# lxa9867/ImageFolder

Hardware: NVIDIA H100
Metric: tokenizer_train_images_per_sec_256x256 (higher is better)
Workload: dtype bf16

## Files before the change

imagefolder_b200/csrc/attn_kernel.cu:

```cuda
#include "xq_common.cuh"
#include "xq_tc.cuh"

#include <mutex>

namespace xq {
using namespace xqtc;

constexpr int AT_BM = 128;
constexpr int AT_BN = 128;
constexpr int AT_D = 64;
constexpr int AT_NS = 2;
constexpr int AT_TILE = AT_BM * AT_D * 2;
constexpr int AT_THREADS = 288;

struct AttnFwdSmem {
    static constexpr int Q = 0;
    static constexpr int K = AT_TILE;
    static constexpr int V = AT_TILE * (1 + AT_NS);
    static constexpr int BAR = AT_TILE * (1 + 2 * AT_NS);
    static constexpr int BYTES = BAR + 256;
};

__device__ __forceinline__ void named_bar_sync(int id, int nthreads) { asm volatile("bar.sync %0, %1;" ::"r"(id), "r"(nthreads) : "memory"); }

__global__ void __launch_bounds__(AT_THREADS, 1)
attn_fwd_kernel(const __grid_constant__ CUtensorMap tmQKV, __nv_bfloat16 *__restrict__ out, float *__restrict__ lse2, int N, int H,
                int nQ , float c ) {
    extern __shared__ uint8_t smem_raw[];
    uint8_t *base = (uint8_t *)(((uintptr_t)smem_raw + 1023) & ~(uintptr_t)1023);
    uint64_t *bars = (uint64_t *)(base + AttnFwdSmem::BAR);
    uint64_t *q_full = bars + 0;
    uint64_t *k_full = bars + 1;
    uint64_t *k_empty = bars + 1 + AT_NS;
    uint64_t *v_full = bars + 1 + 2 * AT_NS;
// ... 22 lines not shown
        for (int j = 0; j < nK; ++j) {
            const int st = j % AT_NS;
            const uint32_t ph = ((j / AT_NS) & 1) ^ 1;
            mbar_wait(&k_empty[st], ph);
            if (elect_one()) {
                mbar_expect_tx(&k_full[st], AT_TILE);
                tma_load_3d(base + AttnFwdSmem::K + st * AT_TILE, &tmQKV, colK, j * AT_BN, b, &k_full[st]);
            }
            __syncwarp();
            mbar_wait(&v_empty[st], ph);
            if (elect_one()) {
                mbar_expect_tx(&v_full[st], AT_TILE);
                tma_load_3d(base + AttnFwdSmem::V + st * AT_TILE, &tmQKV, colV, j * AT_BN, b, &v_full[st]);
            }
            __syncwarp();
        }
        return;
    }

    const int wg = warp >> 2, wq = warp & 3;
    const int rq = wg * 64 + wq * 16 + (lane >> 2), cq = 2 * (lane & 3);
    const uint64_t qd = desc_k_sw128(smem_u32(base + AttnFwdSmem::Q + wg * (AT_TILE / 2)));
    float m[2] = {-CUDART_INF_F, -CUDART_INF_F}, l[2] = {0.f, 0.f};
    float o[32];
#pragma unroll
    for (int i = 0; i < 32; ++i) o[i] = 0.f;
    mbar_wait(q_full, 0);
    for (int j = 0; j < nK; ++j) {
        const int st = j % AT_NS;
        const uint32_t ph = (j / AT_NS) & 1;
        float s[64];
        mbar_wait(&k_full[st], ph);
        const uint64_t kd = desc_k_sw128(smem_u32(base + AttnFwdSmem::K + st * AT_TILE));
        wgmma_fence();
#pragma unroll
        for (int k = 0; k < AT_D / 16; ++k) wgmma_m64n128k16_ss<0, 0>(s, desc_adv(qd, k * 32), desc_adv(kd, k * 32), (uint32_t)k);
        wgmma_commit();
        wgmma_wait<0>();
        fence_regs(s);
        __syncwarp();
        if (lane == 0) mbar_arrive(&k_empty[st]);
        const int nv = N - j * AT_BN;
        if (nv < AT_BN) {
#pragma unroll
            for (int i = 0; i < 64; ++i)
                if (8 * (i >> 2) + cq + (i & 1) >= nv) s[i] = -CUDART_INF_F;
        }
        float mx[2] = {m[0], m[1]};
#pragma unroll
        for (int i = 0; i < 64; ++i) mx[(i >> 1) & 1] = fmaxf(mx[(i >> 1) & 1], s[i]);
#pragma unroll
        for (int hh = 0; hh < 2; ++hh) {
            mx[hh] = fmaxf(mx[hh], __shfl_xor_sync(0xffffffffu, mx[hh], 1));
            mx[hh] = fmaxf(mx[hh], __shfl_xor_sync(0xffffffffu, mx[hh], 2));
        }
        float alpha[2], mc[2];
#pragma unroll
        for (int hh = 0; hh < 2; ++hh) {
            alpha[hh] = ex2_approx((m[hh] - mx[hh]) * c);
            m[hh] = mx[hh];
            mc[hh] = mx[hh] * c;
            l[hh] *= alpha[hh];
        }
#pragma unroll
        for (int i = 0; i < 32; ++i) o[i] *= alpha[(i >> 1) & 1];
        uint32_t pa[AT_BN / 16][4];
#pragma unroll
        for (int i = 0; i < 64; i += 2) {
            const int hh = (i >> 1) & 1;
            const float p0 = ex2_approx(fmaf(s[i], c, -mc[hh])), p1 = ex2_approx(fmaf(s[i + 1], c, -mc[hh]));
            l[hh] += p0 + p1;
            pa[i >> 3][((i >> 2) & 1) * 2 + hh] = pack_bf16(p0, p1);
        }
        mbar_wait(&v_full[st], ph);
        const uint64_t vd = desc_mn_sw128(smem_u32(base + AttnFwdSmem::V + st * AT_TILE), AT_TILE);
        wgmma_fence();
#pragma unroll
        for (int k = 0; k < AT_BN / 16; ++k) wgmma_m64n64k16_rs<1>(o, pa[k], desc_adv(vd, k * 2048), 1u);
        wgmma_commit();
        wgmma_wait<0>();
        fence_regs(o);
        __syncwarp();
        if (lane == 0) mbar_arrive(&v_empty[st]);
    }
#pragma unroll
    for (int hh = 0; hh < 2; ++hh) {
        l[hh] += __shfl_xor_sync(0xffffffffu, l[hh], 1);
        l[hh] += __shfl_xor_sync(0xffffffffu, l[hh], 2);
    }
#pragma unroll
    for (int hh = 0; hh < 2; ++hh) {
        const int n = qt * AT_BM + rq + 8 * hh;
        if (n >= N) continue;
        const float inv = 1.0f / l[hh];
        if (cq == 0) lse2[(size_t)bh * N + n] = fmaf(m[hh], c, log2f(l[hh]));
        __nv_bfloat16 *orow = out + ((size_t)b * N + n) * H * AT_D + h * AT_D;
#pragma unroll
        for (int jj = 0; jj < AT_D / 8; ++jj)
            *reinterpret_cast<uint32_t *>(orow + 8 * jj + cq) = pack_bf16(o[4 * jj + 2 * hh] * inv, o[4 * jj + 2 * hh + 1] * inv);
    }
}

constexpr int AT_TAIL_MAX = 0;

__global__ void __launch_bounds__(128)
attn_fwd_tail_kernel(const __nv_bfloat16 *__restrict__ qkv, __nv_bfloat16 *__restrict__ out, float *__restrict__ lse2, int B, int N,
                     int H, int n0 , float c) {
    const int lane = threadIdx.x & 31;
    const long long w = ((long long)blockIdx.x * blockDim.x + threadIdx.x) >> 5;
    const int nt = N - n0;
    if (w >= (long long)B * H * nt) return;
    const int r = (int)(w % nt);
    const int bh = (int)(w / nt);
    const int b = bh / H, h = bh - b * H;
    const int n = n0 + r;
    const size_t W = (size_t)3 * H * AT_D;
    const __nv_bfloat16 *qp = qkv + ((size_t)b * N + n) * W + h * AT_D;
    float qf[AT_D];
#pragma unroll
    for (int u = 0; u < 8; ++u) {
        const uint4 x = *reinterpret_cast<const uint4 *>(qp + u * 8);
        const __nv_bfloat162 *x2 = reinterpret_cast<const __nv_bfloat162 *>(&x);
#pragma unroll
        for (int e = 0; e < 4; ++e) {
            const float2 f = __bfloat1622float2(x2[e]);
            qf[u * 8 + 2 * e] = f.x * c;
            qf[u * 8 + 2 * e + 1] = f.y * c;
        }
    }
    float m = -CUDART_INF_F, l = 0.f, o[AT_D];
#pragma unroll
    for (int i = 0; i < AT_D; ++i) o[i] = 0.f;
    for (int key = lane; key < N; key += 32) {
        const __nv_bfloat16 *kp = qkv + ((size_t)b * N + key) * W + (H + h) * AT_D;
        const __nv_bfloat16 *vp = kp + (size_t)H * AT_D;
        float s = 0.f;
#pragma unroll
        for (int u = 0; u < 8; ++u) {
            const uint4 x = *reinterpret_cast<const uint4 *>(kp + u * 8);
            const __nv_bfloat162 *x2 = reinterpret_cast<const __nv_bfloat162 *>(&x);
#pragma unroll
            for (int e = 0; e < 4; ++e) {
                const float2 f = __bfloat1622float2(x2[e]);
                s = fmaf(qf[u * 8 + 2 * e], f.x, s);
                s = fmaf(qf[u * 8 + 2 * e + 1], f.y, s);
            }
        }
        const float m_new = fmaxf(m, s);
        const float corr = ex2_approx(m - m_new);
        const float p = ex2_approx(s - m_new);
        l = fmaf(l, corr, p);
        m = m_new;
#pragma unroll
        for (int u = 0; u < 8; ++u) {
            const uint4 x = *reinterpret_cast<const uint4 *>(vp + u * 8);
            const __nv_bfloat162 *x2 = reinterpret_cast<const __nv_bfloat162 *>(&x);
#pragma unroll
            for (int e = 0; e < 4; ++e) {
                const float2 f = __bfloat1622float2(x2[e]);
                o[u * 8 + 2 * e] = fmaf(o[u * 8 + 2 * e], corr, p * f.x);
                o[u * 8 + 2 * e + 1] = fmaf(o[u * 8 + 2 * e + 1], corr, p * f.y);
            }
        }
    }
    float M = m;
#pragma unroll
    for (int off = 16; off > 0; off >>= 1) M = fmaxf(M, __shfl_xor_sync(0xffffffffu, M, off));
    const float f = (m == -CUDART_INF_F) ? 0.f : ex2_approx(m - M);
    l *= f;
#pragma unroll
    for (int off = 16; off > 0; off >>= 1) l += __shfl_xor_sync(0xffffffffu, l, off);
    const float inv = 1.0f / l;
    float mine0 = 0.f, mine1 = 0.f;
#pragma unroll
    for (int i = 0; i < AT_D; ++i) {
        float x = o[i] * f;
#pragma unroll
        for (int off = 16; off > 0; off >>= 1) x += __shfl_xor_sync(0xffffffffu, x, off);
        if (i == 2 * lane) mine0 = x;
        if (i == 2 * lane + 1) mine1 = x;
    }
    __nv_bfloat16 *op = out + ((size_t)b * N + n) * H * AT_D + h * AT_D;
    *reinterpret_cast<uint32_t *>(op + 2 * lane) = pack_bf16(mine0 * inv, mine1 * inv);
    if (lane == 0) lse2[(size_t)bh * N + n] = M + log2f(l);
}

struct AttnMaps {
    const void *qkv;
    int B, N, H;
    CUtensorMap tmQKV;
};

struct AttnDevState { bool fwd_attr = false, bwd_attr = false, prep_attr = false; };
static int attn_dev_state(AttnDevState **out) {
    static std::mutex mu;
    static AttnDevState states[64];
    int dev = 0;
    cudaError_t e = cudaGetDevice(&dev);
    if (e != cudaSuccess) return xq::record_cuda_error(e, "cudaGetDevice");
    if (dev < 0 || dev >= 64) return XQ_ERR_UNSUPPORTED;
    std::lock_guard<std::mutex> g(mu);
    *out = &states[dev];
    return XQ_OK;
}

static bool get_fwd_maps(const void *qkv, int B, int N, int H, AttnMaps &m) {
    static std::mutex mu;
    static AttnMaps cache[16];
    static int n_cached = 0, next = 0;
    std::lock_guard<std::mutex> g(mu);
    for (int i = 0; i < n_cached; ++i)
        if (cache[i].qkv == qkv && cache[i].B == B && cache[i].N == N && cache[i].H == H) { m = cache[i]; return true; }
    AttnMaps e;
    e.qkv = qkv; e.B = B; e.N = N; e.H = H;
    const uint64_t W = (uint64_t)3 * H * AT_D;
    if (!make_map_3d(&e.tmQKV, CU_TENSOR_MAP_DATA_TYPE_BFLOAT16, 2, const_cast<void *>(qkv), W, N, B, W * 2, (uint64_t)N * W * 2, AT_D, AT_BM)) return false;
    cache[next] = e;
    next = (next + 1) % 16;
    if (n_cached < 16) ++n_cached;
    m = e;
    return true;
}


constexpr int AB_THREADS = 288;
constexpr int AB_BQ = 64;
constexpr int AB_QS = 3;
constexpr int AB_QTILE = AB_BQ * AT_D * 2;

struct AttnBwdSmem {
    static constexpr int K = 0;
    static constexpr int V = AT_TILE;
    static constexpr int Q = 2 * AT_TILE;
    static constexpr int DO = Q + AB_QS * AB_QTILE;
    static constexpr int DS = DO + AB_QS * AB_QTILE;
    static constexpr int STAT = DS + 2 * AB_QTILE;
    static constexpr int BAR = STAT + AB_QS * 512;
    static constexpr int BYTES = BAR + 256;
};

__device__ __forceinline__ void bulk_load_1d(void *dst, const void *src, uint32_t bytes, uint64_t *bar) {
    asm volatile("cp.async.bulk.shared::cluster.global.mbarrier::complete_tx::bytes [%0], [%1], %2, [%3];"
                 ::"r"(smem_u32(dst)), "l"(src), "r"(bytes), "r"(smem_u32(bar))
                 : "memory");
}

__device__ __forceinline__ void bwd_epilogue_frag(const float (&acc)[32], float mul, __nv_bfloat16 *__restrict__ row0,
                                                  size_t row_stride, bool ok0, bool ok1, float *__restrict__ g_bias_cols, int lane) {
    const int cq = 2 * (lane & 3);
#pragma unroll
    for (int jj = 0; jj < AT_D / 8; ++jj) {
        const uint32_t w0 = pack_bf16(acc[4 * jj] * mul, acc[4 * jj + 1] * mul);
        const uint32_t w1 = pack_bf16(acc[4 * jj + 2] * mul, acc[4 * jj + 3] * mul);
        if (ok0) *reinterpret_cast<uint32_t *>(row0 + 8 * jj + cq) = w0;
        if (ok1) *reinterpret_cast<uint32_t *>(row0 + 8 * row_stride + 8 * jj + cq) = w1;
        if (g_bias_cols) {
            float s0 = __uint_as_float(w0 << 16) + __uint_as_float(w1 << 16);
            float s1 = __uint_as_float(w0 & 0xffff0000u) + __uint_as_float(w1 & 0xffff0000u);
#pragma unroll
            for (int o = 4; o < 32; o <<= 1) {
                s0 += __shfl_xor_sync(0xffffffffu, s0, o);
                s1 += __shfl_xor_sync(0xffffffffu, s1, o);
            }
            if (lane < 4) {
                atomicAdd(g_bias_cols + 8 * jj + cq, s0);
                atomicAdd(g_bias_cols + 8 * jj + cq + 1, s1);
            }
        }
    }
}

__global__ void __launch_bounds__(AB_THREADS, 1)
attn_bwd_kernel(const __grid_constant__ CUtensorMap tmQKV, const __grid_constant__ CUtensorMap tmDO, const float *__restrict__ lseP,
                const float *__restrict__ deltaP, float *__restrict__ dq_acc, __nv_bfloat16 *__restrict__ dqkv, float *__restrict__ g_bias,
                int N, int H, int Npad, float c, float scale) {
    extern __shared__ uint8_t smem_raw[];
    uint8_t *base = (uint8_t *)(((uintptr_t)smem_raw + 1023) & ~(uintptr_t)1023);
    uint64_t *bars = (uint64_t *)(base + AttnBwdSmem::BAR);
    uint64_t *kv_full = bars;
    uint64_t *q_full = bars + 1;
    uint64_t *q_empty = bars + 1 + AB_QS;
    float *s_lse = (float *)(base + AttnBwdSmem::STAT);
    float *s_delta = s_lse + AB_QS * AB_BQ;

    const int tid = threadIdx.x, warp = tid >> 5, lane = tid & 31;
    const int bh = blockIdx.y, b = bh / H, h = bh - b * H;
    const int k0 = blockIdx.x * AT_BN;
    const int colQ = h * AT_D, colK = (H + h) * AT_D, colV = (2 * H + h) * AT_D;
    const int nQ = (N + AB_BQ - 1) / AB_BQ;

    if (tid == 0) {
        mbar_init(kv_full, 1);
        for (int i = 0; i < AB_QS; ++i) { mbar_init(&q_full[i], 1); mbar_init(&q_empty[i], 8); }
        mbar_fence_init();
    }
    __syncthreads();

// ... 11 lines not shown
        for (int i = 0; i < nQ; ++i) {
            const int st = i % AB_QS;
            mbar_wait(&q_empty[st], ((i / AB_QS) & 1) ^ 1);
            if (elect_one()) {
                mbar_expect_tx(&q_full[st], 2 * AB_QTILE + 2 * AB_BQ * 4);
                tma_load_3d(base + AttnBwdSmem::Q + st * AB_QTILE, &tmQKV, colQ, i * AB_BQ, b, &q_full[st]);
                tma_load_3d(base + AttnBwdSmem::DO + st * AB_QTILE, &tmDO, h * AT_D, i * AB_BQ, b, &q_full[st]);
                bulk_load_1d(s_lse + st * AB_BQ, lseP + (size_t)bh * Npad + i * AB_BQ, AB_BQ * 4, &q_full[st]);
                bulk_load_1d(s_delta + st * AB_BQ, deltaP + (size_t)bh * Npad + i * AB_BQ, AB_BQ * 4, &q_full[st]);
            }
            __syncwarp();
        }
        return;
    }

    const int wg = warp >> 2, wq = warp & 3;
    const int rq = wq * 16 + (lane >> 2), cq = 2 * (lane & 3);
    const int key0 = k0 + wg * 64 + rq;
    const bool kok0 = key0 < N, kok1 = key0 + 8 < N;
    const uint32_t kw = smem_u32(base + AttnBwdSmem::K + wg * AB_QTILE), vw = smem_u32(base + AttnBwdSmem::V + wg * AB_QTILE);
    const uint64_t kd_k = desc_k_sw128(kw), vd_k = desc_k_sw128(vw), kd_mn = desc_mn_sw128(kw, AT_TILE);
    const uint32_t dsw = smem_u32(base + AttnBwdSmem::DS + wg * AB_QTILE);
    const uint64_t dsd = desc_mn_sw128(dsw, AT_TILE);
    float dv[32], dk[32];
#pragma unroll
    for (int i = 0; i < 32; ++i) dv[i] = dk[i] = 0.f;
    mbar_wait(kv_full, 0);
    for (int i = 0; i < nQ; ++i) {
        const int st = i % AB_QS;
        mbar_wait(&q_full[st], (i / AB_QS) & 1);
        const uint32_t qa = smem_u32(base + AttnBwdSmem::Q + st * AB_QTILE), da = smem_u32(base + AttnBwdSmem::DO + st * AB_QTILE);
        float s[32], dp[32];
        wgmma_fence();
#pragma unroll
        for (int k = 0; k < AT_D / 16; ++k) wgmma_m64n64k16_ss<0, 0>(s, desc_adv(kd_k, k * 32), desc_adv(desc_k_sw128(qa), k * 32), (uint32_t)k);
#pragma unroll
        for (int k = 0; k < AT_D / 16; ++k) wgmma_m64n64k16_ss<0, 0>(dp, desc_adv(vd_k, k * 32), desc_adv(desc_k_sw128(da), k * 32), (uint32_t)k);
        wgmma_commit();
        wgmma_wait<0>();
        fence_regs(s);
        fence_regs(dp);
        const float *L = s_lse + st * AB_BQ, *D = s_delta + st * AB_BQ;
        uint32_t pa[4][4], sa[4][4];
#pragma unroll
        for (int jj = 0; jj < AB_BQ / 8; ++jj) {
            const float2 Lq = *reinterpret_cast<const float2 *>(L + 8 * jj + cq);
// ... 11 lines not shown
                sa[jj >> 1][(jj & 1) * 2 + hh] = dw;
                asm volatile("st.shared.b32 [%0], %1;" ::"r"(dsw + rowtile_off_bf16(rq + 8 * hh, 8 * jj + cq)), "r"(dw) : "memory");
            }
        }
        fence_async_smem();
        named_bar_sync(1 + wg, 128);
        const uint64_t qd_mn = desc_mn_sw128(qa, AT_TILE), dd_mn = desc_mn_sw128(da, AT_TILE);
        float dq[32];
        wgmma_fence();
#pragma unroll
        for (int k = 0; k < AB_BQ / 16; ++k) {
            wgmma_m64n64k16_rs<1>(dv, pa[k], desc_adv(dd_mn, k * 2048), 1u);
            wgmma_m64n64k16_rs<1>(dk, sa[k], desc_adv(qd_mn, k * 2048), 1u);
        }
#pragma unroll
        for (int k = 0; k < 64 / 16; ++k) wgmma_m64n64k16_ss<1, 1>(dq, desc_adv(dsd, k * 2048), desc_adv(kd_mn, k * 2048), (uint32_t)k);
        wgmma_commit();
        wgmma_wait<0>();
        fence_regs(dv);
        fence_regs(dk);
        fence_regs(dq);
        __syncwarp();
        if (lane == 0) mbar_arrive(&q_empty[st]);
        named_bar_sync(1 + wg, 128);
#pragma unroll
        for (int hh = 0; hh < 2; ++hh) {
            const int q = i * AB_BQ + rq + 8 * hh;
            if (q < N) {
                float *dst = dq_acc + ((size_t)bh * N + q) * AT_D + cq;
#pragma unroll
                for (int jj = 0; jj < AT_D / 8; ++jj)
                    atomicAdd(reinterpret_cast<float2 *>(dst + 8 * jj), make_float2(dq[4 * jj + 2 * hh], dq[4 * jj + 2 * hh + 1]));
            }
        }
    }
    const size_t W = (size_t)3 * H * AT_D;
    __nv_bfloat16 *row = dqkv + ((size_t)b * N + key0) * W;
    bwd_epilogue_frag(dv, 1.0f, row + colV, W, kok0, kok1, g_bias ? g_bias + colV : nullptr, lane);
    bwd_epilogue_frag(dk, scale, row + colK, W, kok0, kok1, g_bias ? g_bias + colK : nullptr, lane);
}


constexpr int AB_KTAIL_MAX = 4;
constexpr int AB_PREP_ROWS = 128;

__device__ __forceinline__ void unpack8(const uint4 &w, float (&f)[8]) {
    const uint32_t x[4] = {w.x, w.y, w.z, w.w};
#pragma unroll
    for (int e = 0; e < 4; ++e) { f[2 * e] = __uint_as_float(x[e] << 16); f[2 * e + 1] = __uint_as_float(x[e] & 0xffff0000u); }
}

template <int NT>
__global__ void __launch_bounds__(256, 2)
attn_bwd_prep_kernel(const __nv_bfloat16 *__restrict__ qkv, const __nv_bfloat16 *__restrict__ out, const __nv_bfloat16 *__restrict__ dout,
                     const float *__restrict__ lse2, float *__restrict__ lseP, float *__restrict__ deltaP, float *__restrict__ dq_acc,
                     float *__restrict__ dsT, __nv_bfloat16 *__restrict__ dqkv, float *__restrict__ g_bias, int N, int H, int Npad,
                     float c, float scale) {
    constexpr int NTA = NT > 0 ? NT : 1;
// ... 190 lines not shown
        }
    }
    if (!g_bias) return;
#pragma unroll
    for (int e = 0; e < 8; ++e) {
        v[e] += __shfl_xor_sync(0xffffffffu, v[e], 8);
        v[e] += __shfl_xor_sync(0xffffffffu, v[e], 16);
    }
    const int warp = threadIdx.x >> 5, lane = threadIdx.x & 31;
    if (lane < 8) {
#pragma unroll
        for (int e = 0; e < 8; ++e) red[warp][lane * 8 + e] = v[e];
    }
    __syncthreads();
    if (threadIdx.x < AT_D) {
        float acc = 0.f;
#pragma unroll
        for (int w8 = 0; w8 < 8; ++w8) acc += red[w8][threadIdx.x];
        atomicAdd(g_bias + hh * AT_D + threadIdx.x, acc);
    }
}

struct AttnBwdMaps {
    const void *qkv, *dout;
    int B, N, H;
    CUtensorMap tmQKV, tmDO;
};

static bool get_bwd_maps(const void *qkv, const void *dout, int B, int N, int H, AttnBwdMaps &m) {
    static std::mutex mu;
    static AttnBwdMaps cache[16];
    static int n_cached = 0, next = 0;
    std::lock_guard<std::mutex> g(mu);
    for (int i = 0; i < n_cached; ++i)
        if (cache[i].qkv == qkv && cache[i].dout == dout && cache[i].B == B &&
            cache[i].N == N && cache[i].H == H) { m = cache[i]; return true; }
    AttnBwdMaps e;
    e.qkv = qkv; e.dout = dout; e.B = B; e.N = N; e.H = H;
    const uint64_t W = (uint64_t)3 * H * AT_D, Wo = (uint64_t)H * AT_D;
    if (!make_map_3d(&e.tmQKV, CU_TENSOR_MAP_DATA_TYPE_BFLOAT16, 2, const_cast<void *>(qkv), W, N, B, W * 2, (uint64_t)N * W * 2, AT_D, AB_BQ)) return false;
    if (!make_map_3d(&e.tmDO, CU_TENSOR_MAP_DATA_TYPE_BFLOAT16, 2, const_cast<void *>(dout), Wo, N, B, Wo * 2, (uint64_t)N * Wo * 2, AT_D, AB_BQ)) return false;
    cache[next] = e;
    next = (next + 1) % 16;
    if (n_cached < 16) ++n_cached;
    m = e;
    return true;
}

static int attn_bwd_ktail(int N) {
    const int r = N % AT_BN;
    return (N > AT_BN && r != 0 && r <= AB_KTAIL_MAX) ? r : 0;
}

static size_t attn_bwd_ws_layout(int B, int N, int H, size_t *off_lse, size_t *off_delta, size_t *off_dst) {
    const size_t Npad = ((size_t)N + AT_BM - 1) / AT_BM * AT_BM;
    const size_t acc = align_up((size_t)B * H * N * AT_D * sizeof(float), 1024);
    const size_t st = align_up((size_t)B * H * Npad * sizeof(float), 1024);
    const size_t dst = align_up((size_t)B * H * N * attn_bwd_ktail(N) * sizeof(float), 1024);
    if (off_lse) *off_lse = acc;
    if (off_delta) *off_delta = acc + st;
    if (off_dst) *off_dst = acc + 2 * st;
    return acc + 2 * st + dst;
}

// ... 1 lines not shown

extern "C" {

size_t xq_vit_attn_bwd_workspace_bytes(int B, int N, int H) {
    if (B <= 0 || N <= 0 || H <= 0) return 0;
    return xq::attn_bwd_ws_layout(B, N, H, nullptr, nullptr, nullptr);
}

int xq_vit_attn_bwd(const void *qkv, const void *out, const void *d_out, const float *lse2, void *dqkv, float *g_bias, int B, int N,
                    int H, int head_dim, float scale, void *workspace, size_t workspace_bytes, void *stream) {
    using namespace xq;
    if (!qkv || !out || !d_out || !lse2 || !dqkv || !workspace || B <= 0 || N <= 0 || H <= 0) return XQ_ERR_ARG;
    if (head_dim != AT_D) return XQ_ERR_UNSUPPORTED;
    if (((uintptr_t)qkv & 15) || ((uintptr_t)out & 15) || ((uintptr_t)d_out & 15) || ((uintptr_t)dqkv & 15) || ((uintptr_t)workspace & 255))
        return XQ_ERR_ARG;
    size_t off_lse, off_delta, off_dst;
    if (workspace_bytes < attn_bwd_ws_layout(B, N, H, &off_lse, &off_delta, &off_dst)) return XQ_ERR_WORKSPACE;
    cudaStream_t st = (cudaStream_t)stream;
    float *acc = (float *)workspace;
    float *lseP = (float *)((char *)workspace + off_lse);
    float *deltaP = (float *)((char *)workspace + off_delta);
    float *dsT = (float *)((char *)workspace + off_dst);
    AttnBwdMaps m;
    if (!get_bwd_maps(qkv, d_out, B, N, H, m)) return XQ_ERR_UNSUPPORTED;
    const int nt = attn_bwd_ktail(N);
    const int nK = nt ? N / AT_BN : (N + AT_BN - 1) / AT_BN;
    const int Npad = (N + AT_BM - 1) / AT_BM * AT_BM;
    if ((long long)B * H > 65535) return XQ_ERR_UNSUPPORTED;
    if (g_bias) XQ_CUDA_TRY(cudaMemsetAsync(g_bias, 0, (size_t)3 * H * AT_D * sizeof(float), st));
    const float c2 = scale * 1.4426950408889634f;
    AttnDevState *ds = nullptr;
    if (int rc = attn_dev_state(&ds)) return rc;
    {
        dim3 grid(nt ? 1u : (unsigned)(Npad / AB_PREP_ROWS), (unsigned)(B * H));
        const __nv_bfloat16 *qp = (const __nv_bfloat16 *)qkv, *op = (const __nv_bfloat16 *)out, *gp = (const __nv_bfloat16 *)d_out;
        __nv_bfloat16 *dp = (__nv_bfloat16 *)dqkv;
        constexpr int PS = 2 * 3 * (AB_PREP_ROWS / 32) * 256 * 16;
        if (!ds->prep_attr) {
            XQ_CUDA_TRY(cudaFuncSetAttribute(attn_bwd_prep_kernel<1>, cudaFuncAttributeMaxDynamicSharedMemorySize, PS));
            XQ_CUDA_TRY(cudaFuncSetAttribute(attn_bwd_prep_kernel<2>, cudaFuncAttributeMaxDynamicSharedMemorySize, PS));
            XQ_CUDA_TRY(cudaFuncSetAttribute(attn_bwd_prep_kernel<3>, cudaFuncAttributeMaxDynamicSharedMemorySize, PS));
            XQ_CUDA_TRY(cudaFuncSetAttribute(attn_bwd_prep_kernel<4>, cudaFuncAttributeMaxDynamicSharedMemorySize, PS));
            ds->prep_attr = true;
        }
        switch (nt) {
        case 0: attn_bwd_prep_kernel<0><<<grid, 256, 0, st>>>(qp, op, gp, lse2, lseP, deltaP, acc, dsT, dp, g_bias, N, H, Npad, c2, scale); break;
        case 1: attn_bwd_prep_kernel<1><<<grid, 256, PS, st>>>(qp, op, gp, lse2, lseP, deltaP, acc, dsT, dp, g_bias, N, H, Npad, c2, scale); break;
        case 2: attn_bwd_prep_kernel<2><<<grid, 256, PS, st>>>(qp, op, gp, lse2, lseP, deltaP, acc, dsT, dp, g_bias, N, H, Npad, c2, scale); break;
        case 3: attn_bwd_prep_kernel<3><<<grid, 256, PS, st>>>(qp, op, gp, lse2, lseP, deltaP, acc, dsT, dp, g_bias, N, H, Npad, c2, scale); break;
        default: attn_bwd_prep_kernel<4><<<grid, 256, PS, st>>>(qp, op, gp, lse2, lseP, deltaP, acc, dsT, dp, g_bias, N, H, Npad, c2, scale); break;
        }
        XQ_LAUNCH_CHECK("attn_bwd_prep_kernel");
    }
    const size_t smem = AttnBwdSmem::BYTES + 1024;
    if (!ds->bwd_attr) {
        XQ_CUDA_TRY(cudaFuncSetAttribute(attn_bwd_kernel, cudaFuncAttributeMaxDynamicSharedMemorySize, (int)smem));
        ds->bwd_attr = true;
    }
    attn_bwd_kernel<<<dim3((unsigned)nK, (unsigned)(B * H)), AB_THREADS, smem, st>>>(m.tmQKV, m.tmDO, lseP, deltaP, acc,
                                                                                     (__nv_bfloat16 *)dqkv, g_bias, N, H, Npad, c2, scale);
    XQ_LAUNCH_CHECK("attn_bwd_kernel");
    {
        dim3 grid((unsigned)((N + AB_CONV_ROWS - 1) / AB_CONV_ROWS), (unsigned)(B * H));
        attn_dq_convert_kernel<<<grid, 256, 0, st>>>(acc, (const __nv_bfloat16 *)qkv, dsT, (__nv_bfloat16 *)dqkv, g_bias, N, H, N - nt, nt, scale);
        XQ_LAUNCH_CHECK("attn_dq_convert_kernel");
    }
    return XQ_OK;
}

int xq_vit_attn_fwd(const void *qkv, void *out, float *lse2, int B, int N, int H, int head_dim, float scale, void *stream) {
    using namespace xq;
    if (!qkv || !out || !lse2 || B <= 0 || N <= 0 || H <= 0) return XQ_ERR_ARG;
    if (head_dim != AT_D) return XQ_ERR_UNSUPPORTED;
    if (((uintptr_t)qkv & 15) || ((uintptr_t)out & 15)) return XQ_ERR_ARG;
    AttnMaps m;
    if (!get_fwd_maps(qkv, B, N, H, m)) return XQ_ERR_UNSUPPORTED;
    const int n_tail = (N % AT_BM != 0 && N % AT_BM <= AT_TAIL_MAX && N > AT_BM) ? N % AT_BM : 0;
    const int nQ = n_tail ? N / AT_BM : (N + AT_BM - 1) / AT_BM;
    const size_t smem = AttnFwdSmem::BYTES + 1024;
    AttnDevState *ds = nullptr;
    if (int rc = attn_dev_state(&ds)) return rc;
    if (!ds->fwd_attr) {
        XQ_CUDA_TRY(cudaFuncSetAttribute(attn_fwd_kernel, cudaFuncAttributeMaxDynamicSharedMemorySize, (int)smem));
        ds->fwd_attr = true;
    }
    const long long tiles = (long long)B * H * nQ;
    if (tiles > 0x7fffffffLL) return XQ_ERR_ARG;
    const float c = scale * 1.4426950408889634f;
    attn_fwd_kernel<<<(unsigned)tiles, AT_THREADS, smem, (cudaStream_t)stream>>>(m.tmQKV, (__nv_bfloat16 *)out, lse2, N, H, nQ, c);
    XQ_LAUNCH_CHECK("attn_fwd_kernel");
    if (n_tail) {
        const long long warps = (long long)B * H * n_tail;
        attn_fwd_tail_kernel<<<(unsigned)((warps + 3) / 4), 128, 0, (cudaStream_t)stream>>>(
            (const __nv_bfloat16 *)qkv, (__nv_bfloat16 *)out, lse2, B, N, H, N - n_tail, c);
        XQ_LAUNCH_CHECK("attn_fwd_tail_kernel");
    }
    return XQ_OK;
}

}
```

imagefolder_b200/csrc/xq_tc.cuh:

```cuda
#pragma once
#include <cuda.h>
#include <cuda_bf16.h>
#include <cuda_runtime.h>
#include <stdint.h>

namespace xqtc {

__device__ __forceinline__ uint32_t smem_u32(const void *p) { return (uint32_t)__cvta_generic_to_shared(p); }

__device__ __forceinline__ void mbar_init(uint64_t *bar, uint32_t count) {
    asm volatile("mbarrier.init.shared::cta.b64 [%0], %1;" ::"r"(smem_u32(bar)), "r"(count));
}
__device__ __forceinline__ void mbar_fence_init() { asm volatile("fence.mbarrier_init.release.cluster;" ::: "memory"); }
__device__ __forceinline__ void mbar_expect_tx(uint64_t *bar, uint32_t bytes) {
    asm volatile("mbarrier.arrive.expect_tx.shared::cta.b64 _, [%0], %1;" ::"r"(smem_u32(bar)), "r"(bytes) : "memory");
}
__device__ __forceinline__ void mbar_arrive(uint64_t *bar) {
    asm volatile("mbarrier.arrive.shared::cta.b64 _, [%0];" ::"r"(smem_u32(bar)) : "memory");
}
__device__ __forceinline__ bool mbar_try(uint64_t *bar, uint32_t parity) {
    uint32_t done;
    asm volatile(
        "{\n\t.reg .pred p;\n\t"
        "mbarrier.try_wait.parity.shared::cta.b64 p, [%1], %2;\n\t"
// ... 60 lines not shown
    d |= (uint64_t)(1024 >> 4) << 32;
    d |= (uint64_t)1 << 62;
    return d;
}
__device__ __forceinline__ uint64_t desc_adv(uint64_t d, uint32_t bytes) { return d + (uint64_t)(bytes >> 4); }

__device__ __forceinline__ void wgmma_fence() { asm volatile("wgmma.fence.sync.aligned;" ::: "memory"); }
__device__ __forceinline__ void wgmma_commit() { asm volatile("wgmma.commit_group.sync.aligned;" ::: "memory"); }
template <int N>
__device__ __forceinline__ void wgmma_wait() { asm volatile("wgmma.wait_group.sync.aligned %0;" ::"n"(N) : "memory"); }
template <int N>
__device__ __forceinline__ void fence_regs(float (&d)[N]) {
#pragma unroll
    for (int i = 0; i < N; ++i) asm volatile("" : "+f"(d[i])::"memory");
}

template <int TA, int TB>
__device__ __forceinline__ void wgmma_m64n64k16_ss(float (&d)[32], uint64_t da, uint64_t db, uint32_t acc) {
    asm volatile(
        "{\n\t.reg .pred p;\n\tsetp.ne.b32 p, %34, 0;\n\t"
        "wgmma.mma_async.sync.aligned.m64n64k16.f32.bf16.bf16 "
        "{%0, %1, %2, %3, %4, %5, %6, %7, %8, %9, %10, %11, %12, %13, %14, %15, %16, %17, %18, %19, %20, %21, %22, %23, %24, %25, %26, %27, %28, %29, %30, %31}, %32, %33, p, 1, 1, %35, %36;\n\t}"
        : "+f"(d[0]), "+f"(d[1]), "+f"(d[2]), "+f"(d[3]), "+f"(d[4]), "+f"(d[5]), "+f"(d[6]), "+f"(d[7]), "+f"(d[8]), "+f"(d[9]), "+f"(d[10]), "+f"(d[11]), "+f"(d[12]), "+f"(d[13]), "+f"(d[14]), "+f"(d[15]), "+f"(d[16]), "+f"(d[17]), "+f"(d[18]), "+f"(d[19]), "+f"(d[20]), "+f"(d[21]), "+f"(d[22]), "+f"(d[23]), "+f"(d[24]), "+f"(d[25]), "+f"(d[26]), "+f"(d[27]), "+f"(d[28]), "+f"(d[29]), "+f"(d[30]), "+f"(d[31])
        : "l"(da), "l"(db), "r"(acc), "n"(TA), "n"(TB));
}

template <int TA, int TB>
__device__ __forceinline__ void wgmma_m64n128k16_ss(float (&d)[64], uint64_t da, uint64_t db, uint32_t acc) {
    asm volatile(
        "{\n\t.reg .pred p;\n\tsetp.ne.b32 p, %66, 0;\n\t"
        "wgmma.mma_async.sync.aligned.m64n128k16.f32.bf16.bf16 "
        "{%0, %1, %2, %3, %4, %5, %6, %7, %8, %9, %10, %11, %12, %13, %14, %15, %16, %17, %18, %19, %20, %21, %22, %23, %24, %25, %26, %27, %28, %29, %30, %31, %32, %33, %34, %35, %36, %37, %38, %39, %40, %41, %42, %43, %44, %45, %46, %47, %48, %49, %50, %51, %52, %53, %54, %55, %56, %57, %58, %59, %60, %61, %62, %63}, %64, %65, p, 1, 1, %67, %68;\n\t}"
        : "+f"(d[0]), "+f"(d[1]), "+f"(d[2]), "+f"(d[3]), "+f"(d[4]), "+f"(d[5]), "+f"(d[6]), "+f"(d[7]), "+f"(d[8]), "+f"(d[9]), "+f"(d[10]), "+f"(d[11]), "+f"(d[12]), "+f"(d[13]), "+f"(d[14]), "+f"(d[15]), "+f"(d[16]), "+f"(d[17]), "+f"(d[18]), "+f"(d[19]), "+f"(d[20]), "+f"(d[21]), "+f"(d[22]), "+f"(d[23]), "+f"(d[24]), "+f"(d[25]), "+f"(d[26]), "+f"(d[27]), "+f"(d[28]), "+f"(d[29]), "+f"(d[30]), "+f"(d[31]), "+f"(d[32]), "+f"(d[33]), "+f"(d[34]), "+f"(d[35]), "+f"(d[36]), "+f"(d[37]), "+f"(d[38]), "+f"(d[39]), "+f"(d[40]), "+f"(d[41]), "+f"(d[42]), "+f"(d[43]), "+f"(d[44]), "+f"(d[45]), "+f"(d[46]), "+f"(d[47]), "+f"(d[48]), "+f"(d[49]), "+f"(d[50]), "+f"(d[51]), "+f"(d[52]), "+f"(d[53]), "+f"(d[54]), "+f"(d[55]), "+f"(d[56]), "+f"(d[57]), "+f"(d[58]), "+f"(d[59]), "+f"(d[60]), "+f"(d[61]), "+f"(d[62]), "+f"(d[63])
        : "l"(da), "l"(db), "r"(acc), "n"(TA), "n"(TB));
}

template <int TB>
__device__ __forceinline__ void wgmma_m64n64k16_rs(float (&d)[32], const uint32_t (&a)[4], uint64_t db, uint32_t acc) {
    asm volatile(
        "{\n\t.reg .pred p;\n\tsetp.ne.b32 p, %37, 0;\n\t"
        "wgmma.mma_async.sync.aligned.m64n64k16.f32.bf16.bf16 "
        "{%0, %1, %2, %3, %4, %5, %6, %7, %8, %9, %10, %11, %12, %13, %14, %15, %16, %17, %18, %19, %20, %21, %22, %23, %24, %25, %26, %27, %28, %29, %30, %31}, {%32, %33, %34, %35}, %36, p, 1, 1, %38;\n\t}"
        : "+f"(d[0]), "+f"(d[1]), "+f"(d[2]), "+f"(d[3]), "+f"(d[4]), "+f"(d[5]), "+f"(d[6]), "+f"(d[7]), "+f"(d[8]), "+f"(d[9]), "+f"(d[10]), "+f"(d[11]), "+f"(d[12]), "+f"(d[13]), "+f"(d[14]), "+f"(d[15]), "+f"(d[16]), "+f"(d[17]), "+f"(d[18]), "+f"(d[19]), "+f"(d[20]), "+f"(d[21]), "+f"(d[22]), "+f"(d[23]), "+f"(d[24]), "+f"(d[25]), "+f"(d[26]), "+f"(d[27]), "+f"(d[28]), "+f"(d[29]), "+f"(d[30]), "+f"(d[31])
        : "r"(a[0]), "r"(a[1]), "r"(a[2]), "r"(a[3]), "l"(db), "r"(acc), "n"(TB));
}

// ... 72 lines not shown
```

Before: 472.6.

## Overlap QK and PV wgmma in attention forward, TMA-reduce dQ in backward

The forward consumer loop is software-pipelined so that the S=QK^T wgmma for block j is issued together with the PV wgmma for block j-1, overlapping softmax with tensor-core work. The K/V ring buffer grows from two to three stages. A narrow-width tail path (n64/n16 wgmma) replaces the separate scalar tail kernel. In the backward pass, per-element float atomics for dQ are replaced by a swizzled shared-memory staging tile and TMA bulk reduce-add, which uses more shared memory and adds bulk-async waits.

```diff
diff --git a/imagefolder_b200/csrc/attn_kernel.cu b/imagefolder_b200/csrc/attn_kernel.cu
--- a/imagefolder_b200/csrc/attn_kernel.cu
+++ b/imagefolder_b200/csrc/attn_kernel.cu
@@ -2,6 +2,7 @@
 #include "xq_tc.cuh"
 
 #include <mutex>
+#include <type_traits>
 
 namespace xq {
 using namespace xqtc;
@@ -9,7 +10,7 @@
 constexpr int AT_BM = 128;
 constexpr int AT_BN = 128;
 constexpr int AT_D = 64;
-constexpr int AT_NS = 2;
+constexpr int AT_NS = 3;
 constexpr int AT_TILE = AT_BM * AT_D * 2;
 constexpr int AT_THREADS = 288;
 
@@ -78,25 +79,22 @@
     const int rq = wg * 64 + wq * 16 + (lane >> 2), cq = 2 * (lane & 3);
     const uint64_t qd = desc_k_sw128(smem_u32(base + AttnFwdSmem::Q + wg * (AT_TILE / 2)));
     float m[2] = {-CUDART_INF_F, -CUDART_INF_F}, l[2] = {0.f, 0.f};
-    float o[32];
+    float o[32], s[64], alpha[2];
 #pragma unroll
     for (int i = 0; i < 32; ++i) o[i] = 0.f;
-    mbar_wait(q_full, 0);
-    for (int j = 0; j < nK; ++j) {
-        const int st = j % AT_NS;
-        const uint32_t ph = (j / AT_NS) & 1;
-        float s[64];
-        mbar_wait(&k_full[st], ph);
-        const uint64_t kd = desc_k_sw128(smem_u32(base + AttnFwdSmem::K + st * AT_TILE));
-        wgmma_fence();
+    uint32_t pa[AT_BN / 16][4];
+    auto kdesc = [&](int j) { return desc_k_sw128(smem_u32(base + AttnFwdSmem::K + (j % AT_NS) * AT_TILE)); };
+    auto vdesc = [&](int j) { return desc_mn_sw128(smem_u32(base + AttnFwdSmem::V + (j % AT_NS) * AT_TILE), AT_TILE); };
+    auto release = [&](uint64_t *empty, int j) { __syncwarp(); if (lane == 0) mbar_arrive(&empty[j % AT_NS]); };
+    auto issue_s128 = [&](uint64_t kd) {
 #pragma unroll
         for (int k = 0; k < AT_D / 16; ++k) wgmma_m64n128k16_ss<0, 0>(s, desc_adv(qd, k * 32), desc_adv(kd, k * 32), (uint32_t)k);
-        wgmma_commit();
-        wgmma_wait<0>();
-        fence_regs(s);
-        __syncwarp();
-        if (lane == 0) mbar_arrive(&k_empty[st]);
-        const int nv = N - j * AT_BN;
+    };
+    auto issue_pv = [&](uint64_t vd, int ksteps) {
+#pragma unroll
+        for (int k = 0; k < ksteps; ++k) wgmma_m64n64k16_rs<1>(o, pa[k], desc_adv(vd, k * 2048), 1u);
+    };
+    auto softmax = [&](int nv) {
         if (nv < AT_BN) {
 #pragma unroll
             for (int i = 0; i < 64; ++i)
@@ -110,7 +108,7 @@
             mx[hh] = fmaxf(mx[hh], __shfl_xor_sync(0xffffffffu, mx[hh], 1));
             mx[hh] = fmaxf(mx[hh], __shfl_xor_sync(0xffffffffu, mx[hh], 2));
         }
-        float alpha[2], mc[2];
+        float mc[2];
 #pragma unroll
         for (int hh = 0; hh < 2; ++hh) {
             alpha[hh] = ex2_approx((m[hh] - mx[hh]) * c);
@@ -119,25 +117,93 @@
             l[hh] *= alpha[hh];
         }
 #pragma unroll
-        for (int i = 0; i < 32; ++i) o[i] *= alpha[(i >> 1) & 1];
-        uint32_t pa[AT_BN / 16][4];
-#pragma unroll
         for (int i = 0; i < 64; i += 2) {
             const int hh = (i >> 1) & 1;
-            const float p0 = ex2_approx(fmaf(s[i], c, -mc[hh])), p1 = ex2_approx(fmaf(s[i + 1], c, -mc[hh]));
-            l[hh] += p0 + p1;
-            pa[i >> 3][((i >> 2) & 1) * 2 + hh] = pack_bf16(p0, p1);
-        }
-        mbar_wait(&v_full[st], ph);
-        const uint64_t vd = desc_mn_sw128(smem_u32(base + AttnFwdSmem::V + st * AT_TILE), AT_TILE);
+            s[i] = ex2_approx(fmaf(s[i], c, -mc[hh]));
+            s[i + 1] = ex2_approx(fmaf(s[i + 1], c, -mc[hh]));
+            l[hh] += s[i] + s[i + 1];
+        }
+    };
+    auto rescale_pack = [&]() {
+#pragma unroll
+        for (int i = 0; i < 32; ++i) o[i] *= alpha[(i >> 1) & 1];
+#pragma unroll
+        for (int i = 0; i < 64; i += 2)
+            pa[i >> 3][((i >> 2) & 1) * 2 + ((i >> 1) & 1)] = pack_bf16(s[i], s[i + 1]);
+    };
+
+    const int tailk = (nK > 1) ? N % AT_BN : 0;
+    const int nKm = nK - (tailk ? 1 : 0);
+    mbar_wait(q_full, 0);
+    mbar_wait(&k_full[0], 0);
+    wgmma_fence();
+    issue_s128(kdesc(0));
+    wgmma_commit();
+    wgmma_wait<0>();
+    fence_regs(s);
+    release(k_empty, 0);
+    softmax(N);
+    rescale_pack();
+    for (int j = 1; j < nKm; ++j) {
+        mbar_wait(&v_full[(j - 1) % AT_NS], ((j - 1) / AT_NS) & 1);
+        mbar_wait(&k_full[j % AT_NS], (j / AT_NS) & 1);
         wgmma_fence();
-#pragma unroll
-        for (int k = 0; k < AT_BN / 16; ++k) wgmma_m64n64k16_rs<1>(o, pa[k], desc_adv(vd, k * 2048), 1u);
+        issue_s128(kdesc(j));
+        wgmma_commit();
+        issue_pv(vdesc(j - 1), AT_BN / 16);
+        wgmma_commit();
+        wgmma_wait<1>();
+        fence_regs(s);
+        release(k_empty, j);
+        softmax(AT_BN);
+        wgmma_wait<0>();
+        fence_regs(o);
+        release(v_empty, j - 1);
+        rescale_pack();
+    }
+    auto tail_block = [&](auto width) {
+        constexpr int W = decltype(width)::value;
+        const int j = nK - 1;
+        const uint64_t kd = kdesc(j);
+        wgmma_fence();
+#pragma unroll
+        for (int k = 0; k < AT_D / 16; ++k) {
+            if constexpr (W == 128) wgmma_m64n128k16_ss<0, 0>(s, desc_adv(qd, k * 32), desc_adv(kd, k * 32), (uint32_t)k);
+            else if constexpr (W == 64) wgmma_m64n64k16_ss<0, 0>(reinterpret_cast<float(&)[32]>(s[0]), desc_adv(qd, k * 32), desc_adv(kd, k * 32), (uint32_t)k);
+            else wgmma_m64n16k16_ss<0, 0>(reinterpret_cast<float(&)[8]>(s[0]), desc_adv(qd, k * 32), desc_adv(kd, k * 32), (uint32_t)k);
+        }
+        issue_pv(vdesc(j - 1), AT_BN / 16);
+        wgmma_commit();
+        wgmma_wait<0>();
+        fence_regs(s);
+        fence_regs(o);
+        release(k_empty, j);
+        release(v_empty, j - 1);
+        softmax(tailk);
+        rescale_pack();
+        mbar_wait(&v_full[j % AT_NS], (j / AT_NS) & 1);
+        wgmma_fence();
+        issue_pv(vdesc(j), W / 16);
         wgmma_commit();
         wgmma_wait<0>();
         fence_regs(o);
-        __syncwarp();
-        if (lane == 0) mbar_arrive(&v_empty[st]);
+        release(v_empty, j);
+    };
+    if (tailk) {
+        const int j = nK - 1;
+        mbar_wait(&v_full[(j - 1) % AT_NS], ((j - 1) / AT_NS) & 1);
+        mbar_wait(&k_full[j % AT_NS], (j / AT_NS) & 1);
+        if (tailk > 64) tail_block(std::integral_constant<int, 128>());
+        else if (tailk > 16) tail_block(std::integral_constant<int, 64>());
+        else tail_block(std::integral_constant<int, 16>());
+    } else {
+        mbar_wait(&v_full[(nK - 1) % AT_NS], ((nK - 1) / AT_NS) & 1);
+        wgmma_fence();
+        issue_pv(vdesc(nK - 1), AT_BN / 16);
+        wgmma_commit();
+        wgmma_wait<0>();
+        fence_regs(o);
+        release(v_empty, nK - 1);
     }
 #pragma unroll
     for (int hh = 0; hh < 2; ++hh) {
@@ -155,90 +221,6 @@
         for (int jj = 0; jj < AT_D / 8; ++jj)
             *reinterpret_cast<uint32_t *>(orow + 8 * jj + cq) = pack_bf16(o[4 * jj + 2 * hh] * inv, o[4 * jj + 2 * hh + 1] * inv);
     }
-}
-
-constexpr int AT_TAIL_MAX = 0;
-
-__global__ void __launch_bounds__(128)
-attn_fwd_tail_kernel(const __nv_bfloat16 *__restrict__ qkv, __nv_bfloat16 *__restrict__ out, float *__restrict__ lse2, int B, int N,
-                     int H, int n0 , float c) {
-    const int lane = threadIdx.x & 31;
-    const long long w = ((long long)blockIdx.x * blockDim.x + threadIdx.x) >> 5;
-    const int nt = N - n0;
-    if (w >= (long long)B * H * nt) return;
-    const int r = (int)(w % nt);
-    const int bh = (int)(w / nt);
-    const int b = bh / H, h = bh - b * H;
-    const int n = n0 + r;
-    const size_t W = (size_t)3 * H * AT_D;
-    const __nv_bfloat16 *qp = qkv + ((size_t)b * N + n) * W + h * AT_D;
-    float qf[AT_D];
-#pragma unroll
-    for (int u = 0; u < 8; ++u) {
-        const uint4 x = *reinterpret_cast<const uint4 *>(qp + u * 8);
-        const __nv_bfloat162 *x2 = reinterpret_cast<const __nv_bfloat162 *>(&x);
-#pragma unroll
-        for (int e = 0; e < 4; ++e) {
-            const float2 f = __bfloat1622float2(x2[e]);
-            qf[u * 8 + 2 * e] = f.x * c;
-            qf[u * 8 + 2 * e + 1] = f.y * c;
-        }
-    }
-    float m = -CUDART_INF_F, l = 0.f, o[AT_D];
-#pragma unroll
-    for (int i = 0; i < AT_D; ++i) o[i] = 0.f;
-    for (int key = lane; key < N; key += 32) {
-        const __nv_bfloat16 *kp = qkv + ((size_t)b * N + key) * W + (H + h) * AT_D;
-        const __nv_bfloat16 *vp = kp + (size_t)H * AT_D;
-        float s = 0.f;
-#pragma unroll
-        for (int u = 0; u < 8; ++u) {
-            const uint4 x = *reinterpret_cast<const uint4 *>(kp + u * 8);
-            const __nv_bfloat162 *x2 = reinterpret_cast<const __nv_bfloat162 *>(&x);
-#pragma unroll
-            for (int e = 0; e < 4; ++e) {
-                const float2 f = __bfloat1622float2(x2[e]);
-                s = fmaf(qf[u * 8 + 2 * e], f.x, s);
-                s = fmaf(qf[u * 8 + 2 * e + 1], f.y, s);
-            }
-        }
-        const float m_new = fmaxf(m, s);
-        const float corr = ex2_approx(m - m_new);
-        const float p = ex2_approx(s - m_new);
-        l = fmaf(l, corr, p);
-        m = m_new;
-#pragma unroll
-        for (int u = 0; u < 8; ++u) {
-            const uint4 x = *reinterpret_cast<const uint4 *>(vp + u * 8);
-            const __nv_bfloat162 *x2 = reinterpret_cast<const __nv_bfloat162 *>(&x);
-#pragma unroll
-            for (int e = 0; e < 4; ++e) {
-                const float2 f = __bfloat1622float2(x2[e]);
-                o[u * 8 + 2 * e] = fmaf(o[u * 8 + 2 * e], corr, p * f.x);
-                o[u * 8 + 2 * e + 1] = fmaf(o[u * 8 + 2 * e + 1], corr, p * f.y);
-            }
-        }
-    }
-    float M = m;
-#pragma unroll
-    for (int off = 16; off > 0; off >>= 1) M = fmaxf(M, __shfl_xor_sync(0xffffffffu, M, off));
-    const float f = (m == -CUDART_INF_F) ? 0.f : ex2_approx(m - M);
-    l *= f;
-#pragma unroll
-    for (int off = 16; off > 0; off >>= 1) l += __shfl_xor_sync(0xffffffffu, l, off);
-    const float inv = 1.0f / l;
-    float mine0 = 0.f, mine1 = 0.f;
-#pragma unroll
-    for (int i = 0; i < AT_D; ++i) {
-        float x = o[i] * f;
-#pragma unroll
-        for (int off = 16; off > 0; off >>= 1) x += __shfl_xor_sync(0xffffffffu, x, off);
-        if (i == 2 * lane) mine0 = x;
-        if (i == 2 * lane + 1) mine1 = x;
-    }
-    __nv_bfloat16 *op = out + ((size_t)b * N + n) * H * AT_D + h * AT_D;
-    *reinterpret_cast<uint32_t *>(op + 2 * lane) = pack_bf16(mine0 * inv, mine1 * inv);
-    if (lane == 0) lse2[(size_t)bh * N + n] = M + log2f(l);
 }
 
 struct AttnMaps {
@@ -283,6 +265,11 @@
 constexpr int AB_BQ = 64;
 constexpr int AB_QS = 3;
 constexpr int AB_QTILE = AB_BQ * AT_D * 2;
+constexpr int AB_DQTILE = AB_BQ * AT_D * 4;
+
+__device__ __forceinline__ uint32_t dqtile_off(int r, int c) {
+    return (uint32_t)((c >> 5) * (AB_DQTILE / 2) + r * 128 + (((((c & 31) >> 2) ^ (r & 7)) & 7) << 4) + (c & 3) * 4);
+}
 
 struct AttnBwdSmem {
     static constexpr int K = 0;
@@ -290,7 +277,8 @@
     static constexpr int Q = 2 * AT_TILE;
     static constexpr int DO = Q + AB_QS * AB_QTILE;
     static constexpr int DS = DO + AB_QS * AB_QTILE;
-    static constexpr int STAT = DS + 2 * AB_QTILE;
+    static constexpr int DQ = DS + 2 * AB_QTILE;
+    static constexpr int STAT = DQ + 2 * AB_DQTILE;
     static constexpr int BAR = STAT + AB_QS * 512;
     static constexpr int BYTES = BAR + 256;
 };
@@ -327,8 +315,8 @@
 }
 
 __global__ void __launch_bounds__(AB_THREADS, 1)
-attn_bwd_kernel(const __grid_constant__ CUtensorMap tmQKV, const __grid_constant__ CUtensorMap tmDO, const float *__restrict__ lseP,
-                const float *__restrict__ deltaP, float *__restrict__ dq_acc, __nv_bfloat16 *__restrict__ dqkv, float *__restrict__ g_bias,
+attn_bwd_kernel(const __grid_constant__ CUtensorMap tmQKV, const __grid_constant__ CUtensorMap tmDO, const __grid_constant__ CUtensorMap tmDQ,
+                const float *__restrict__ lseP, const float *__restrict__ deltaP, __nv_bfloat16 *__restrict__ dqkv, float *__restrict__ g_bias,
                 int N, int H, int Npad, float c, float scale) {
     extern __shared__ uint8_t smem_raw[];
     uint8_t *base = (uint8_t *)(((uintptr_t)smem_raw + 1023) & ~(uintptr_t)1023);
@@ -386,6 +374,9 @@
     const uint64_t kd_k = desc_k_sw128(kw), vd_k = desc_k_sw128(vw), kd_mn = desc_mn_sw128(kw, AT_TILE);
     const uint32_t dsw = smem_u32(base + AttnBwdSmem::DS + wg * AB_QTILE);
     const uint64_t dsd = desc_mn_sw128(dsw, AT_TILE);
+    uint8_t *dqt = base + AttnBwdSmem::DQ + wg * AB_DQTILE;
+    const uint32_t dqw = smem_u32(dqt);
+    const bool leader = (tid & 127) == 0;
     float dv[32], dk[32];
 #pragma unroll
     for (int i = 0; i < 32; ++i) dv[i] = dk[i] = 0.f;
@@ -443,18 +434,24 @@
         fence_regs(dq);
         __syncwarp();
         if (lane == 0) mbar_arrive(&q_empty[st]);
+        if (leader) bulk_wait_read<0>();
         named_bar_sync(1 + wg, 128);
 #pragma unroll
         for (int hh = 0; hh < 2; ++hh) {
-            const int q = i * AB_BQ + rq + 8 * hh;
-            if (q < N) {
-                float *dst = dq_acc + ((size_t)bh * N + q) * AT_D + cq;
-#pragma unroll
-                for (int jj = 0; jj < AT_D / 8; ++jj)
-                    atomicAdd(reinterpret_cast<float2 *>(dst + 8 * jj), make_float2(dq[4 * jj + 2 * hh], dq[4 * jj + 2 * hh + 1]));
-            }
-        }
-    }
+#pragma unroll
+            for (int jj = 0; jj < AT_D / 8; ++jj)
+                asm volatile("st.shared.v2.f32 [%0], {%1, %2};" ::"r"(dqw + dqtile_off(rq + 8 * hh, 8 * jj + cq)),
+                             "f"(dq[4 * jj + 2 * hh]), "f"(dq[4 * jj + 2 * hh + 1]) : "memory");
+        }
+        fence_async_smem();
+        named_bar_sync(1 + wg, 128);
+        if (leader) {
+            tma_reduce_add_3d(&tmDQ, dqt, 0, i * AB_BQ, bh);
+            tma_reduce_add_3d(&tmDQ, dqt + AB_DQTILE / 2, 32, i * AB_BQ, bh);
+            bulk_commit();
+        }
+    }
+    if (leader) bulk_wait<0>();
     const size_t W = (size_t)3 * H * AT_D;
     __nv_bfloat16 *row = dqkv + ((size_t)b * N + key0) * W;
     bwd_epilogue_frag(dv, 1.0f, row + colV, W, kok0, kok1, g_bias ? g_bias + colV : nullptr, lane);
@@ -691,24 +688,25 @@
 }
 
 struct AttnBwdMaps {
-    const void *qkv, *dout;
+    const void *qkv, *dout, *acc;
     int B, N, H;
-    CUtensorMap tmQKV, tmDO;
+    CUtensorMap tmQKV, tmDO, tmDQ;
 };
 
-static bool get_bwd_maps(const void *qkv, const void *dout, int B, int N, int H, AttnBwdMaps &m) {
+static bool get_bwd_maps(const void *qkv, const void *dout, void *acc, int B, int N, int H, AttnBwdMaps &m) {
     static std::mutex mu;
     static AttnBwdMaps cache[16];
     static int n_cached = 0, next = 0;
     std::lock_guard<std::mutex> g(mu);
     for (int i = 0; i < n_cached; ++i)
-        if (cache[i].qkv == qkv && cache[i].dout == dout && cache[i].B == B &&
+        if (cache[i].qkv == qkv && cache[i].dout == dout && cache[i].acc == acc && cache[i].B == B &&
             cache[i].N == N && cache[i].H == H) { m = cache[i]; return true; }
     AttnBwdMaps e;
-    e.qkv = qkv; e.dout = dout; e.B = B; e.N = N; e.H = H;
+    e.qkv = qkv; e.dout = dout; e.acc = acc; e.B = B; e.N = N; e.H = H;
     const uint64_t W = (uint64_t)3 * H * AT_D, Wo = (uint64_t)H * AT_D;
     if (!make_map_3d(&e.tmQKV, CU_TENSOR_MAP_DATA_TYPE_BFLOAT16, 2, const_cast<void *>(qkv), W, N, B, W * 2, (uint64_t)N * W * 2, AT_D, AB_BQ)) return false;
     if (!make_map_3d(&e.tmDO, CU_TENSOR_MAP_DATA_TYPE_BFLOAT16, 2, const_cast<void *>(dout), Wo, N, B, Wo * 2, (uint64_t)N * Wo * 2, AT_D, AB_BQ)) return false;
+    if (!make_map_3d(&e.tmDQ, CU_TENSOR_MAP_DATA_TYPE_FLOAT32, 4, acc, AT_D, N, (uint64_t)B * H, AT_D * 4, (uint64_t)N * AT_D * 4, 32, AB_BQ)) return false;
     cache[next] = e;
     next = (next + 1) % 16;
     if (n_cached < 16) ++n_cached;
@@ -756,7 +754,7 @@
     float *deltaP = (float *)((char *)workspace + off_delta);
     float *dsT = (float *)((char *)workspace + off_dst);
     AttnBwdMaps m;
-    if (!get_bwd_maps(qkv, d_out, B, N, H, m)) return XQ_ERR_UNSUPPORTED;
+    if (!get_bwd_maps(qkv, d_out, acc, B, N, H, m)) return XQ_ERR_UNSUPPORTED;
     const int nt = attn_bwd_ktail(N);
     const int nK = nt ? N / AT_BN : (N + AT_BN - 1) / AT_BN;
     const int Npad = (N + AT_BM - 1) / AT_BM * AT_BM;
@@ -791,7 +789,7 @@
         XQ_CUDA_TRY(cudaFuncSetAttribute(attn_bwd_kernel, cudaFuncAttributeMaxDynamicSharedMemorySize, (int)smem));
         ds->bwd_attr = true;
     }
-    attn_bwd_kernel<<<dim3((unsigned)nK, (unsigned)(B * H)), AB_THREADS, smem, st>>>(m.tmQKV, m.tmDO, lseP, deltaP, acc,
+    attn_bwd_kernel<<<dim3((unsigned)nK, (unsigned)(B * H)), AB_THREADS, smem, st>>>(m.tmQKV, m.tmDO, m.tmDQ, lseP, deltaP,
                                                                                      (__nv_bfloat16 *)dqkv, g_bias, N, H, Npad, c2, scale);
     XQ_LAUNCH_CHECK("attn_bwd_kernel");
     {
@@ -809,8 +807,7 @@
     if (((uintptr_t)qkv & 15) || ((uintptr_t)out & 15)) return XQ_ERR_ARG;
     AttnMaps m;
     if (!get_fwd_maps(qkv, B, N, H, m)) return XQ_ERR_UNSUPPORTED;
-    const int n_tail = (N % AT_BM != 0 && N % AT_BM <= AT_TAIL_MAX && N > AT_BM) ? N % AT_BM : 0;
-    const int nQ = n_tail ? N / AT_BM : (N + AT_BM - 1) / AT_BM;
+    const int nQ = (N + AT_BM - 1) / AT_BM;
     const size_t smem = AttnFwdSmem::BYTES + 1024;
     AttnDevState *ds = nullptr;
     if (int rc = attn_dev_state(&ds)) return rc;
@@ -823,12 +820,6 @@
     const float c = scale * 1.4426950408889634f;
     attn_fwd_kernel<<<(unsigned)tiles, AT_THREADS, smem, (cudaStream_t)stream>>>(m.tmQKV, (__nv_bfloat16 *)out, lse2, N, H, nQ, c);
     XQ_LAUNCH_CHECK("attn_fwd_kernel");
-    if (n_tail) {
-        const long long warps = (long long)B * H * n_tail;
-        attn_fwd_tail_kernel<<<(unsigned)((warps + 3) / 4), 128, 0, (cudaStream_t)stream>>>(
-            (const __nv_bfloat16 *)qkv, (__nv_bfloat16 *)out, lse2, B, N, H, N - n_tail, c);
-        XQ_LAUNCH_CHECK("attn_fwd_tail_kernel");
-    }
     return XQ_OK;
 }
 
diff --git a/imagefolder_b200/csrc/xq_tc.cuh b/imagefolder_b200/csrc/xq_tc.cuh
--- a/imagefolder_b200/csrc/xq_tc.cuh
+++ b/imagefolder_b200/csrc/xq_tc.cuh
@@ -106,6 +106,16 @@
         "wgmma.mma_async.sync.aligned.m64n64k16.f32.bf16.bf16 "
         "{%0, %1, %2, %3, %4, %5, %6, %7, %8, %9, %10, %11, %12, %13, %14, %15, %16, %17, %18, %19, %20, %21, %22, %23, %24, %25, %26, %27, %28, %29, %30, %31}, %32, %33, p, 1, 1, %35, %36;\n\t}"
         : "+f"(d[0]), "+f"(d[1]), "+f"(d[2]), "+f"(d[3]), "+f"(d[4]), "+f"(d[5]), "+f"(d[6]), "+f"(d[7]), "+f"(d[8]), "+f"(d[9]), "+f"(d[10]), "+f"(d[11]), "+f"(d[12]), "+f"(d[13]), "+f"(d[14]), "+f"(d[15]), "+f"(d[16]), "+f"(d[17]), "+f"(d[18]), "+f"(d[19]), "+f"(d[20]), "+f"(d[21]), "+f"(d[22]), "+f"(d[23]), "+f"(d[24]), "+f"(d[25]), "+f"(d[26]), "+f"(d[27]), "+f"(d[28]), "+f"(d[29]), "+f"(d[30]), "+f"(d[31])
+        : "l"(da), "l"(db), "r"(acc), "n"(TA), "n"(TB));
+}
+
+template <int TA, int TB>
+__device__ __forceinline__ void wgmma_m64n16k16_ss(float (&d)[8], uint64_t da, uint64_t db, uint32_t acc) {
+    asm volatile(
+        "{\n\t.reg .pred p;\n\tsetp.ne.b32 p, %10, 0;\n\t"
+        "wgmma.mma_async.sync.aligned.m64n16k16.f32.bf16.bf16 "
+        "{%0, %1, %2, %3, %4, %5, %6, %7}, %8, %9, p, 1, 1, %11, %12;\n\t}"
+        : "+f"(d[0]), "+f"(d[1]), "+f"(d[2]), "+f"(d[3]), "+f"(d[4]), "+f"(d[5]), "+f"(d[6]), "+f"(d[7])
         : "l"(da), "l"(db), "r"(acc), "n"(TA), "n"(TB));
 }
 
```

New measurement: 482.9, median of 6. 1.02x the previous value.
